# lorenlugosch/end-to-end-SLU

Measured on AMD Instinct MI355X. Metric: utterances/sec (train step, 3 s @16 kHz, B=64), higher is better.
Workload: dtype f32 (trainable stages: exact fp32 MFMA; convolutions and GRU contractions of FROZEN stages: bf16x3 = every fp32 operand split EXACTLY into 3 bf16 terms (3 x 8 = 24 significand bits, fp32's exponent range), 6 bf16 MFMA products per fp32 product (only terms below 2^-24 |a b| dropped), fp32 accumulatio; 1 GPU; experiments/no_unfreezing.cfg SLU train step (frozen SincNet/conv/biGRU encoder in train mode + intent biGRU trained): fwd + 3-slot CE + bwd + grad all-reduce + Adam; batch_per_gpu=64, global_batch=64, samples_per_utterance=48000, parallelism=dp1, encoder_lookahead_batches=20

## Files before the change

end-to-end-slu_amd/csrc/slu_head.hip:

```cpp
#include "slu_common.h"
#include "slu_philox.h"

#include <algorithm>

namespace slu {

constexpr int HEAD_THREADS = 256;
constexpr int HEAD_MAX_SLOTS = 8;

struct HeadParams {
  const float* h;
  const float* W;
  const float* bias;
  const long long* y;
  float* logits;
  int* argmax_t;
  long long* pred;
  float* d_logits;
  float* row_stats;
  float* loss_acc;
  double* epoch_sums;
  unsigned int* ticket;
  int T, B, C, V, S;
  int w_in_lds;
  int vec;
  float drop_p, drop_scale;
  unsigned long long seed, offset;
  const unsigned long long* offset_dev;
  float* h_drop;
  int slot_begin[HEAD_MAX_SLOTS + 1];
};

template <bool COHERENT>
__device__ __forceinline__ void head_reduce_body(const float* row_stats, float* loss_acc, double* epoch_sums, int B) {
  __shared__ float r0[256], r1[256];
  float a = 0.0f, c = 0.0f;
  for (int b = threadIdx.x; b < B; b += 256) {
    if (COHERENT) {
      const unsigned long long g = __hip_atomic_load(reinterpret_cast<const unsigned long long*>(row_stats) + b,
                                                     __ATOMIC_RELAXED, __HIP_MEMORY_SCOPE_AGENT);
      a += __uint_as_float((unsigned)(g & 0xffffffffull));
      c += __uint_as_float((unsigned)(g >> 32));
    } else {
      a += row_stats[2 * b]; c += row_stats[2 * b + 1];
    }
  }
  r0[threadIdx.x] = a; r1[threadIdx.x] = c;
  __syncthreads();
  for (int o = 128; o > 0; o >>= 1) {
    if ((int)threadIdx.x < o) { r0[threadIdx.x] += r0[threadIdx.x + o]; r1[threadIdx.x] += r1[threadIdx.x + o]; }
    __syncthreads();
  }
  if (threadIdx.x == 0) {
    const float loss = r0[0] / (float)B, acc = r1[0] / (float)B;
    loss_acc[0] = loss; loss_acc[1] = acc;
    if (epoch_sums) { epoch_sums[0] += (double)loss * (double)B; epoch_sums[1] += (double)acc * (double)B; }
  }
}

__global__ void __launch_bounds__(256)
head_reduce_kernel(const float* __restrict__ row_stats, float* __restrict__ loss_acc, double* epoch_sums, int B) {
  head_reduce_body<false>(row_stats, loss_acc, epoch_sums, B);
}

__global__ void __launch_bounds__(HEAD_THREADS)
head_fwd_kernel(const HeadParams p) {
  extern __shared__ __attribute__((aligned(16))) char smem[];
  float* sh = reinterpret_cast<float*>(smem);
  float* sw = sh + (size_t)p.T * (p.C + 1);
  float* sl = sw + (p.w_in_lds ? (size_t)p.V * (p.C + 1) : 0);
  float* sm = sl + (size_t)p.T * p.V;
  const int b = blockIdx.x, tid = threadIdx.x;
  const int T = p.T, C = p.C, V = p.V, LD = p.C + 1;
  if (p.vec) {
    const int C4 = C >> 2;
    const int nh = T * C4, nw = p.w_in_lds ? V * C4 : 0;
    const float thr = 1.0f - p.drop_p;
    const unsigned long long off = p.offset + (p.offset_dev ? *p.offset_dev : 0ull);
    constexpr int U = 13;
    for (int base = 0; base < nh + nw; base += HEAD_THREADS * U) {
      float4 v[U];
#pragma unroll
      for (int j = 0; j < U; ++j) {
        const int idx = base + j * HEAD_THREADS + tid;
        const bool ok = idx < nh + nw, isw = idx >= nh;
        const int e = ok ? (isw ? idx - nh : idx) : 0;
        const int row = e / C4, c = (e - row * C4) * 4;
        const float* src = (ok && isw) ? p.W + (size_t)row * C + c : p.h + ((size_t)row * p.B + b) * C + c;
        v[j] = *reinterpret_cast<const float4*>(src);
      }
#pragma unroll
      for (int j = 0; j < U; ++j) {
        const int idx = base + j * HEAD_THREADS + tid;
        const bool ok = idx < nh + nw, isw = idx >= nh;
        const int e = ok ? (isw ? idx - nh : idx) : 0;
        const int row = e / C4, c = (e - row * C4) * 4;
        if (!ok) continue;
        float4 x = v[j];
        if (!isw && p.drop_p > 0.0f) {
          const size_t g = ((size_t)row * p.B + b) * C + c;
          const float4 k = philox_keep4(p.seed, off, g, thr, p.drop_scale);
          x = make_float4(x.x * k.x, x.y * k.y, x.z * k.z, x.w * k.w);
          if (p.h_drop) *reinterpret_cast<float4*>(p.h_drop + g) = x;
        }
        float* dst = sh + (isw ? T + row : row) * LD + c;
        dst[0] = x.x; dst[1] = x.y; dst[2] = x.z; dst[3] = x.w;
      }
    }
  } else {
    const int nh = T * C, nw = p.w_in_lds ? V * C : 0;
    constexpr int U = 48;
    for (int base = 0; base < nh + nw; base += HEAD_THREADS * U) {
      float v[U];
#pragma unroll
      for (int j = 0; j < U; ++j) {
        const int idx = base + j * HEAD_THREADS + tid;
        const bool ok = idx < nh + nw, isw = idx >= nh;
        const int e = ok ? (isw ? idx - nh : idx) : 0;
        const int row = e / C, c = e - row * C;
        const float* src = (ok && isw) ? p.W + e : p.h + ((size_t)row * p.B + b) * C + c;
        v[j] = *src;
      }
#pragma unroll
      for (int j = 0; j < U; ++j) {
        const int idx = base + j * HEAD_THREADS + tid;
        const bool ok = idx < nh + nw, isw = idx >= nh;
        const int e = ok ? (isw ? idx - nh : idx) : 0;
        const int row = e / C, c = e - row * C;
        if (ok) sh[(isw ? T + row : row) * LD + c] = v[j];
      }
    }
  }
  __syncthreads();
  {
    const int lane = tid & 63, wave = tid >> 6;
    const int i = lane & 15, kg = lane >> 4;
    const int MT = (T + 15) >> 4, NT = (V + 15) >> 4;
    for (int tile = wave; tile < MT * NT; tile += HEAD_THREADS / 64) {
      const int mt = tile / NT, nt = tile - mt * NT;
      const float* a = sh + min(mt * 16 + i, T - 1) * LD + kg;
      const int vb = min(nt * 16 + i, V - 1);
      const float* w = (p.w_in_lds ? sw + vb * LD : p.W + (size_t)vb * C) + kg;
      f32x4 acc = {0.f, 0.f, 0.f, 0.f};
      int k0 = 0;
      for (; k0 + 31 < C; k0 += 32) {
        float av[8], bv[8];
#pragma unroll
        for (int u = 0; u < 8; ++u) { av[u] = a[k0 + 4 * u]; bv[u] = w[k0 + 4 * u]; }
#pragma unroll
        for (int u = 0; u < 8; ++u) acc = mfma16(av[u], bv[u], acc);
      }
      for (; k0 < C; k0 += 4) {
        const bool ok = k0 + kg < C;
        acc = mfma16(ok ? a[k0] : 0.0f, ok ? w[k0] : 0.0f, acc);
      }
#pragma unroll
      for (int r = 0; r < 4; ++r) {
        const int t = mt * 16 + 4 * kg + r, v = nt * 16 + i;
        if (t < T && v < V) sl[t * V + v] = acc[r] + p.bias[v];
      }
    }
  }
  __syncthreads();
  if (tid < V) {
    float best = sl[tid];
    int arg = 0;
    for (int t = 1; t < T; ++t) {
      const float x = sl[t * V + tid];
      if (x > best) { best = x; arg = t; }
    }
    sm[tid] = best;
    p.logits[(size_t)b * V + tid] = best;
    p.argmax_t[(size_t)b * V + tid] = arg;
  }
  __syncthreads();
  __shared__ float s_part[HEAD_THREADS];
  __shared__ int s_ok[HEAD_THREADS];
  if (tid < V) {
    int sl_ = 0;
    while (sl_ + 1 < p.S && tid >= p.slot_begin[sl_ + 1]) ++sl_;
    const int v0 = p.slot_begin[sl_], v1 = p.slot_begin[sl_ + 1];
    float mx = sm[v0];
    int am = v0;
    for (int v = v0 + 1; v < v1; ++v) if (sm[v] > mx) { mx = sm[v]; am = v; }
    if (tid == v0) p.pred[(size_t)b * p.S + sl_] = am - v0;
    s_part[tid] = 0.0f;
    s_ok[tid] = 1;
    if (p.y) {
      float den = 0.0f;
      for (int v = v0; v < v1; ++v) den += expf(sm[v] - mx);
      const int yv = (int)p.y[(size_t)b * p.S + sl_];
      if (tid == v0) {
        s_part[tid] = logf(den) - (sm[v0 + yv] - mx);
        s_ok[tid] = (am - v0 == yv) ? 1 : 0;
      }
      if (p.d_logits) {
        const float inv = 1.0f / (den * (float)p.B);
        p.d_logits[(size_t)b * V + tid] = expf(sm[tid] - mx) * inv - ((tid - v0 == yv) ? 1.0f / (float)p.B : 0.0f);
      }
    }
  }
  __syncthreads();
  if (tid == 0 && p.y) {
    float loss = 0.0f;
    bool all_ok = true;
    for (int s2 = 0; s2 < p.S; ++s2) {
      loss += s_part[p.slot_begin[s2]];
      all_ok = all_ok && (s_ok[p.slot_begin[s2]] != 0);
    }
    const unsigned long long g = (unsigned long long)__float_as_uint(loss) |
                                 ((unsigned long long)__float_as_uint(all_ok ? 1.0f : 0.0f) << 32);
    __hip_atomic_store(reinterpret_cast<unsigned long long*>(p.row_stats) + b, g, __ATOMIC_RELAXED, __HIP_MEMORY_SCOPE_AGENT);
  }
  if (p.ticket && p.y) {
    __shared__ int s_last;
    if (tid == 0) {
      asm volatile("s_waitcnt vmcnt(0)" ::: "memory");
      s_last = (__hip_atomic_fetch_add(p.ticket, 1u, __ATOMIC_RELAXED, __HIP_MEMORY_SCOPE_AGENT) == gridDim.x - 1) ? 1 : 0;
    }
    __syncthreads();
    if (s_last) {
      head_reduce_body<true>(p.row_stats, p.loss_acc, p.epoch_sums, p.B);
      if (tid == 0) *p.ticket = 0u;
    }
  }
}

struct HeadDrop {
  float p, scale;
  unsigned long long seed, offset;
  const unsigned long long* offset_dev;
};

__device__ __forceinline__ void
head_bwd_dh_body(char* smem, const int b, const float* __restrict__ d_logits, const int* __restrict__ argmax_t,
                 const float* __restrict__ W, const float* __restrict__ gscale,
                 float* __restrict__ d_h, int T, int B, int C, int V, const HeadDrop& dr) {
  float* acc = reinterpret_cast<float*>(smem);
  __shared__ float s_dl[HEAD_THREADS];
  __shared__ int s_at[HEAD_THREADS];
  const int tid = threadIdx.x;
  const float g = gscale[0];
  if (tid < V) { s_dl[tid] = d_logits[(size_t)b * V + tid] * g; s_at[tid] = argmax_t[(size_t)b * V + tid]; }
  for (int idx = tid; idx < T * C; idx += HEAD_THREADS) acc[idx] = 0.0f;
  __syncthreads();
  for (int c = tid; c < C; c += HEAD_THREADS)
    for (int v = 0; v < V; ++v) acc[s_at[v] * C + c] = fmaf(s_dl[v], W[(size_t)v * C + c], acc[s_at[v] * C + c]);
  __syncthreads();
  if (dr.p > 0.0f) {
    const int C4 = C >> 2;
    const float thr = 1.0f - dr.p;
    const unsigned long long off = dr.offset + (dr.offset_dev ? *dr.offset_dev : 0ull);
    for (int idx = tid; idx < T * C4; idx += HEAD_THREADS) {
      const int t = idx / C4, c = (idx - t * C4) * 4;
      const size_t g = ((size_t)t * B + b) * C + c;
      const float4 k = philox_keep4(dr.seed, off, g, thr, dr.scale);
      const float* a = acc + t * C + c;
      *reinterpret_cast<float4*>(d_h + g) = make_float4(a[0] * k.x, a[1] * k.y, a[2] * k.z, a[3] * k.w);
    }
    return;
  }
  for (int idx = tid; idx < T * C; idx += HEAD_THREADS) {
    const int t = idx / C, c = idx - t * C;
    d_h[((size_t)t * B + b) * C + c] = acc[idx];
  }
}

__device__ __forceinline__ void
head_bwd_dw_body(char* smem, const int v, const float* __restrict__ d_logits, const int* __restrict__ argmax_t,
                 const float* __restrict__ h, const float* __restrict__ gscale,
                 float* __restrict__ d_W, float* __restrict__ d_bias, int T, int B, int C, int V) {
  float* part = reinterpret_cast<float*>(smem);
  float* s_dl = part + 4 * C;
  int* s_at = reinterpret_cast<int*>(s_dl + HEAD_THREADS);
  __shared__ float s_b[4];
  const int lane = threadIdx.x & 63, w = threadIdx.x >> 6;
  const float g = gscale[0];
  float bsum = 0.0f;
  constexpr int KMAX = 16;
  float acc[KMAX];
#pragma unroll
  for (int k = 0; k < KMAX; ++k) acc[k] = 0.0f;
  for (int bb = 0; bb < B; bb += HEAD_THREADS) {
    __syncthreads();
    if (bb + (int)threadIdx.x < B) {
      s_dl[threadIdx.x] = d_logits[(size_t)(bb + threadIdx.x) * V + v];
      s_at[threadIdx.x] = argmax_t[(size_t)(bb + threadIdx.x) * V + v];
    }
    __syncthreads();
    const int nb = min(HEAD_THREADS, B - bb);
    for (int bl0 = w; bl0 < nb; bl0 += 32) {
      float hv[8][KMAX > 4 ? 4 : KMAX];
      if (C <= 256) {
#pragma unroll
        for (int u = 0; u < 8; ++u) {
          const int bl = min(bl0 + 4 * u, nb - 1);
          const float* hr = h + ((size_t)s_at[bl] * B + (bb + bl)) * C;
#pragma unroll
          for (int k = 0; k < 4; ++k) hv[u][k] = hr[min(lane + 64 * k, C - 1)];
        }
#pragma unroll
        for (int u = 0; u < 8; ++u) {
          const int bl = bl0 + 4 * u;
          if (bl < nb) {
            const float dl = s_dl[bl];
            bsum += dl;
#pragma unroll
            for (int k = 0; k < 4; ++k)
              if (lane + 64 * k < C) acc[k] = fmaf(dl, hv[u][k], acc[k]);
          }
        }
      } else {
        for (int u = 0; u < 8; ++u) {
          const int bl = bl0 + 4 * u;
          if (bl >= nb) break;
          const float dl = s_dl[bl];
          const float* hr = h + ((size_t)s_at[bl] * B + (bb + bl)) * C;
          bsum += dl;
#pragma unroll
          for (int k = 0; k < KMAX; ++k) {
            const int c = lane + 64 * k;
            if (c < C) acc[k] = fmaf(dl, hr[c], acc[k]);
          }
        }
      }
    }
  }
#pragma unroll
  for (int k = 0; k < KMAX; ++k) {
    const int c = lane + 64 * k;
    if (c < C) part[w * C + c] = acc[k];
  }
  if (lane == 0) s_b[w] = bsum;
  __syncthreads();
  for (int c = threadIdx.x; c < C; c += HEAD_THREADS)
    d_W[(size_t)v * C + c] = (((part[c] + part[C + c]) + part[2 * C + c]) + part[3 * C + c]) * g;
  if (threadIdx.x == 0) d_bias[v] = (((s_b[0] + s_b[1]) + s_b[2]) + s_b[3]) * g;
  (void)T;
}

__global__ void __launch_bounds__(HEAD_THREADS)
head_bwd_kernel(const float* __restrict__ d_logits, const int* __restrict__ argmax_t, const float* __restrict__ h,
                const float* __restrict__ W, const float* __restrict__ gscale, float* __restrict__ d_h,
                float* __restrict__ d_W, float* __restrict__ d_bias, int n_dh, int T, int B, int C, int V,
                const HeadDrop dr) {
  extern __shared__ __attribute__((aligned(16))) char smem[];
  if ((int)blockIdx.x < n_dh)
    head_bwd_dh_body(smem, blockIdx.x, d_logits, argmax_t, W, gscale, d_h, T, B, C, V, dr);
  else
    head_bwd_dw_body(smem, (int)blockIdx.x - n_dh, d_logits, argmax_t, h, gscale, d_W, d_bias, T, B, C, V);
}

}

using namespace slu;

extern "C" int slu_cls_maxpool_ce_fwd(const float* h, const float* weight, const float* bias,
                                      const int64_t* y, const int64_t* values_per_slot,
                                      int64_t num_slots, float* logits, int32_t* argmax_t,
                                      int64_t* pred, float* d_logits, float* row_stats,
                                      float* loss_acc, double* epoch_sums, uint32_t* ticket, float drop_p,
                                      uint64_t drop_seed, uint64_t drop_offset, const uint64_t* drop_offset_dev,
                                      float* h_drop, int64_t T, int64_t B, int64_t C, void* stream) {
  SLU_REQUIRE(h && weight && bias && logits && argmax_t && pred && values_per_slot, "slu_cls_maxpool_ce_fwd: null pointer");
  SLU_REQUIRE(drop_p >= 0.0f && drop_p < 1.0f, "slu_cls_maxpool_ce_fwd: dropout probability must be in [0, 1)");
  SLU_REQUIRE(num_slots >= 1 && num_slots <= HEAD_MAX_SLOTS, "slu_cls_maxpool_ce_fwd: 1..%d slots supported", HEAD_MAX_SLOTS);
  SLU_REQUIRE(!y || (row_stats && loss_acc), "slu_cls_maxpool_ce_fwd: row_stats / loss_acc required with labels");
  SLU_REQUIRE(T > 0 && B > 0 && C > 0, "slu_cls_maxpool_ce_fwd: non-positive size");
  HeadParams p;
  p.h = h; p.W = weight; p.bias = bias; p.y = (const long long*)y; p.logits = logits; p.argmax_t = argmax_t;
  p.pred = (long long*)pred; p.d_logits = d_logits; p.row_stats = row_stats;
  p.loss_acc = loss_acc; p.epoch_sums = y ? epoch_sums : nullptr; p.ticket = (unsigned int*)ticket;
  p.T = (int)T; p.B = (int)B; p.C = (int)C; p.S = (int)num_slots;
  p.vec = ((C & 3) == 0 && (((uintptr_t)h | (uintptr_t)weight | (uintptr_t)h_drop) & 15) == 0) ? 1 : 0;
  if (drop_p > 0.0f && !p.vec)
    SLU_FAIL(SLU_ERR_UNSUPPORTED, "slu_cls_maxpool_ce_fwd: the fused dropout needs C %% 4 == 0 (got %lld) and 16-byte aligned "
             "h / weight / h_drop", (long long)C);
  p.drop_p = drop_p; p.drop_scale = drop_p > 0.0f ? 1.0f / (1.0f - drop_p) : 1.0f;
  p.seed = drop_seed; p.offset = drop_offset; p.offset_dev = (const unsigned long long*)drop_offset_dev;
  p.h_drop = drop_p > 0.0f ? h_drop : nullptr;
  int V = 0;
  for (int s = 0; s < num_slots; ++s) { p.slot_begin[s] = V; V += (int)values_per_slot[s]; }
  p.slot_begin[num_slots] = V;
  p.V = V;
  SLU_REQUIRE(V >= 1 && V <= HEAD_THREADS, "slu_cls_maxpool_ce_fwd: 1..%d classifier outputs supported", HEAD_THREADS);
  size_t lds = ((size_t)(T + V) * (C + 1) + (size_t)T * V + V) * sizeof(float);
  p.w_in_lds = 1;
  const size_t lds_cap = 160 * 1024 - 4096;
  if (lds > lds_cap) {
    p.w_in_lds = 0;
    lds = ((size_t)T * (C + 1) + (size_t)T * V + V) * sizeof(float);
  }
  if (lds > lds_cap) SLU_FAIL(SLU_ERR_UNSUPPORTED, "slu_cls_maxpool_ce_fwd: T=%lld x C=%lld does not fit the LDS", (long long)T, (long long)C);
  if (lds > 64 * 1024) {
    hipError_t e = hipFuncSetAttribute((const void*)head_fwd_kernel, hipFuncAttributeMaxDynamicSharedMemorySize, (int)lds);
    if (e != hipSuccess) SLU_FAIL(SLU_ERR_HIP, "slu_cls_maxpool_ce_fwd: %s", hipGetErrorString(e));
  }
  hipStream_t st = (hipStream_t)stream;
  hipLaunchKernelGGL(head_fwd_kernel, dim3((unsigned)B), dim3(HEAD_THREADS), lds, st, p);
  SLU_CHECK_LAUNCH("head_fwd_kernel");
  if (y && !ticket) {
    hipLaunchKernelGGL(head_reduce_kernel, dim3(1), dim3(256), 0, st, (const float*)row_stats, loss_acc, epoch_sums, (int)B);
    SLU_CHECK_LAUNCH("head_reduce_kernel");
  }
  return SLU_OK;
}

extern "C" int slu_cls_maxpool_ce_bwd(const float* d_logits, const int32_t* argmax_t, const float* h,
                                      const float* weight, const float* grad_scale, float* d_h,
                                      float* d_weight, float* d_bias, float drop_p, uint64_t drop_seed,
                                      uint64_t drop_offset, const uint64_t* drop_offset_dev, int64_t T, int64_t B,
                                      int64_t C, int64_t V, void* stream) {
  SLU_REQUIRE(d_logits && argmax_t && h && weight && grad_scale, "slu_cls_maxpool_ce_bwd: null pointer");
  SLU_REQUIRE(drop_p >= 0.0f && drop_p < 1.0f, "slu_cls_maxpool_ce_bwd: dropout probability must be in [0, 1)");
  if (drop_p > 0.0f && d_h && ((C & 3) || ((uintptr_t)d_h & 15)))
    SLU_FAIL(SLU_ERR_UNSUPPORTED, "slu_cls_maxpool_ce_bwd: the fused dropout needs C %% 4 == 0 and a 16-byte aligned d_h");
  HeadDrop dr;
  dr.p = drop_p; dr.scale = drop_p > 0.0f ? 1.0f / (1.0f - drop_p) : 1.0f;
  dr.seed = drop_seed; dr.offset = drop_offset; dr.offset_dev = (const unsigned long long*)drop_offset_dev;
  SLU_REQUIRE((d_weight == nullptr) == (d_bias == nullptr), "slu_cls_maxpool_ce_bwd: d_weight and d_bias go together");
  SLU_REQUIRE(C <= 1024, "slu_cls_maxpool_ce_bwd: C <= 1024");
  hipStream_t st = (hipStream_t)stream;
  size_t lds = 0;
  if (d_h) {
    SLU_REQUIRE(V <= HEAD_THREADS && T * C * 4 <= 160 * 1024 - 4096, "slu_cls_maxpool_ce_bwd: T*C too large for the LDS");
    lds = (size_t)T * C * sizeof(float);
  }
  if (d_weight) lds = std::max(lds, ((size_t)4 * C + 2 * HEAD_THREADS) * sizeof(float));
  if (!d_h && !d_weight) return SLU_OK;
  if (lds > 64 * 1024) {
    hipError_t e = hipFuncSetAttribute((const void*)head_bwd_kernel, hipFuncAttributeMaxDynamicSharedMemorySize, (int)lds);
    if (e != hipSuccess) SLU_FAIL(SLU_ERR_HIP, "slu_cls_maxpool_ce_bwd: %s", hipGetErrorString(e));
  }
  const int n_dh = d_h ? (int)B : 0;
  hipLaunchKernelGGL(head_bwd_kernel, dim3((unsigned)(n_dh + (d_weight ? V : 0))), dim3(HEAD_THREADS), lds, st,
                     d_logits, argmax_t, h, weight, grad_scale, d_h, d_weight, d_bias, n_dh, (int)T, (int)B, (int)C, (int)V, dr);
  SLU_CHECK_LAUNCH("head_bwd_kernel");
  return SLU_OK;
}
```

Before: 376,700 utterances/s.

## Add fast head forward path with interleaved LDS layout and fused max-pool

Adds a templated fast variant of the classifier head forward kernel for small T, V and C. It stores h and W in LDS with a permuted, padded row layout so each lane can issue float4 loads feeding the fp32 MFMA. The loads are software-pipelined, and the max-over-time reduction is fused into the MFMA epilogue with cross-lane shuffles instead of writing the full T x V logits to LDS. The path is gated on shape conditions and can be turned off with an environment variable. This adds a second code path and assumes that at most two M tiles and two N tiles cover the work.

```diff
diff --git a/end-to-end-slu_amd/csrc/slu_head.hip b/end-to-end-slu_amd/csrc/slu_head.hip
--- a/end-to-end-slu_amd/csrc/slu_head.hip
+++ b/end-to-end-slu_amd/csrc/slu_head.hip
@@ -2,6 +2,7 @@
 #include "slu_philox.h"
 
 #include <algorithm>
+#include <cstdlib>
 
 namespace slu {
 
@@ -63,15 +64,17 @@
   head_reduce_body<false>(row_stats, loss_acc, epoch_sums, B);
 }
 
+template <bool FAST>
 __global__ void __launch_bounds__(HEAD_THREADS)
 head_fwd_kernel(const HeadParams p) {
   extern __shared__ __attribute__((aligned(16))) char smem[];
+  const int LD = FAST ? p.C + 4 : p.C + 1;
   float* sh = reinterpret_cast<float*>(smem);
-  float* sw = sh + (size_t)p.T * (p.C + 1);
-  float* sl = sw + (p.w_in_lds ? (size_t)p.V * (p.C + 1) : 0);
-  float* sm = sl + (size_t)p.T * p.V;
+  float* sw = sh + (size_t)p.T * LD;
+  float* sl = sw + (p.w_in_lds ? (size_t)p.V * LD : 0);
+  float* sm = sl + (FAST ? 128 : (size_t)p.T * p.V);
   const int b = blockIdx.x, tid = threadIdx.x;
-  const int T = p.T, C = p.C, V = p.V, LD = p.C + 1;
+  const int T = p.T, C = p.C, V = p.V;
   if (p.vec) {
     const int C4 = C >> 2;
     const int nh = T * C4, nw = p.w_in_lds ? V * C4 : 0;
@@ -103,8 +106,13 @@
           x = make_float4(x.x * k.x, x.y * k.y, x.z * k.z, x.w * k.w);
           if (p.h_drop) *reinterpret_cast<float4*>(p.h_drop + g) = x;
         }
-        float* dst = sh + (isw ? T + row : row) * LD + c;
-        dst[0] = x.x; dst[1] = x.y; dst[2] = x.z; dst[3] = x.w;
+        if (FAST) {
+          float* dst = sh + (isw ? T + row : row) * LD + (c & ~15) + ((c >> 2) & 3);
+          dst[0] = x.x; dst[4] = x.y; dst[8] = x.z; dst[12] = x.w;
+        } else {
+          float* dst = sh + (isw ? T + row : row) * LD + c;
+          dst[0] = x.x; dst[1] = x.y; dst[2] = x.z; dst[3] = x.w;
+        }
       }
     }
   } else {
@@ -132,7 +140,45 @@
     }
   }
   __syncthreads();
-  {
+  if (FAST) {
+    const int lane = tid & 63, wave = tid >> 6;
+    const int i = lane & 15, kg = lane >> 4;
+    const int MT = (T + 15) >> 4, NT = (V + 15) >> 4;
+    if (wave < MT * NT) {
+      const int mt = wave / NT, nt = wave - mt * NT;
+      const int vb = min(nt * 16 + i, V - 1);
+      const float4* a = reinterpret_cast<const float4*>(sh + min(mt * 16 + i, T - 1) * LD + 4 * kg);
+      const float4* w = reinterpret_cast<const float4*>(sw + vb * LD + 4 * kg);
+      const int nj = C >> 4;
+      f32x4 acc = {0.f, 0.f, 0.f, 0.f};
+      float4 a0 = a[0], w0 = w[0], a1 = a[4], w1 = w[4];
+      for (int j = 0; j < nj; j += 2) {
+        const int jn = min(j + 2, nj - 2);
+        const float4 a2 = a[4 * jn], w2 = w[4 * jn], a3 = a[4 * jn + 4], w3 = w[4 * jn + 4];
+        acc = mfma16(a0.x, w0.x, acc); acc = mfma16(a0.y, w0.y, acc); acc = mfma16(a0.z, w0.z, acc); acc = mfma16(a0.w, w0.w, acc);
+        acc = mfma16(a1.x, w1.x, acc); acc = mfma16(a1.y, w1.y, acc); acc = mfma16(a1.z, w1.z, acc); acc = mfma16(a1.w, w1.w, acc);
+        a0 = a2; w0 = w2; a1 = a3; w1 = w3;
+      }
+      const float bias = p.bias[vb];
+      float best = acc[0] + bias;
+      int arg = mt * 16 + 4 * kg;
+#pragma unroll
+      for (int r = 1; r < 4; ++r) {
+        const float x = acc[r] + bias;
+        if (x > best) { best = x; arg = mt * 16 + 4 * kg + r; }
+      }
+#pragma unroll
+      for (int o = 16; o < 64; o <<= 1) {
+        const float ob = __shfl_xor(best, o);
+        const int oa = __shfl_xor(arg, o);
+        if (ob > best || (ob == best && oa < arg)) { best = ob; arg = oa; }
+      }
+      if (kg == 0 && nt * 16 + i < V) {
+        sl[mt * 32 + nt * 16 + i] = best;
+        reinterpret_cast<int*>(sl)[64 + mt * 32 + nt * 16 + i] = arg;
+      }
+    }
+  } else {
     const int lane = tid & 63, wave = tid >> 6;
     const int i = lane & 15, kg = lane >> 4;
     const int MT = (T + 15) >> 4, NT = (V + 15) >> 4;
@@ -165,9 +211,14 @@
   if (tid < V) {
     float best = sl[tid];
     int arg = 0;
-    for (int t = 1; t < T; ++t) {
-      const float x = sl[t * V + tid];
-      if (x > best) { best = x; arg = t; }
+    if (FAST) {
+      arg = reinterpret_cast<const int*>(sl)[64 + tid];
+      if (T > 16 && sl[32 + tid] > best) { best = sl[32 + tid]; arg = reinterpret_cast<const int*>(sl)[96 + tid]; }
+    } else {
+      for (int t = 1; t < T; ++t) {
+        const float x = sl[t * V + tid];
+        if (x > best) { best = x; arg = t; }
+      }
     }
     sm[tid] = best;
     p.logits[(size_t)b * V + tid] = best;
@@ -386,18 +437,26 @@
   SLU_REQUIRE(V >= 1 && V <= HEAD_THREADS, "slu_cls_maxpool_ce_fwd: 1..%d classifier outputs supported", HEAD_THREADS);
   size_t lds = ((size_t)(T + V) * (C + 1) + (size_t)T * V + V) * sizeof(float);
   p.w_in_lds = 1;
+  bool fast = p.vec && (C & 31) == 0 && C <= 512 && T <= 32 && V <= 32;
+  if (fast) {
+    const char* env = getenv("SLU_HEAD_FAST");
+    fast = !(env && atoi(env) == 0);
+  }
+  if (fast) lds = ((size_t)(T + V) * (C + 4) + 128 + V) * sizeof(float);
   const size_t lds_cap = 160 * 1024 - 4096;
   if (lds > lds_cap) {
     p.w_in_lds = 0;
     lds = ((size_t)T * (C + 1) + (size_t)T * V + V) * sizeof(float);
   }
   if (lds > lds_cap) SLU_FAIL(SLU_ERR_UNSUPPORTED, "slu_cls_maxpool_ce_fwd: T=%lld x C=%lld does not fit the LDS", (long long)T, (long long)C);
+  const void* kernel = fast ? (const void*)head_fwd_kernel<true> : (const void*)head_fwd_kernel<false>;
   if (lds > 64 * 1024) {
-    hipError_t e = hipFuncSetAttribute((const void*)head_fwd_kernel, hipFuncAttributeMaxDynamicSharedMemorySize, (int)lds);
+    hipError_t e = hipFuncSetAttribute(kernel, hipFuncAttributeMaxDynamicSharedMemorySize, (int)lds);
     if (e != hipSuccess) SLU_FAIL(SLU_ERR_HIP, "slu_cls_maxpool_ce_fwd: %s", hipGetErrorString(e));
   }
   hipStream_t st = (hipStream_t)stream;
-  hipLaunchKernelGGL(head_fwd_kernel, dim3((unsigned)B), dim3(HEAD_THREADS), lds, st, p);
+  if (fast) hipLaunchKernelGGL(head_fwd_kernel<true>, dim3((unsigned)B), dim3(HEAD_THREADS), lds, st, p);
+  else hipLaunchKernelGGL(head_fwd_kernel<false>, dim3((unsigned)B), dim3(HEAD_THREADS), lds, st, p);
   SLU_CHECK_LAUNCH("head_fwd_kernel");
   if (y && !ticket) {
     hipLaunchKernelGGL(head_reduce_kernel, dim3(1), dim3(256), 0, st, (const float*)row_stats, loss_acc, epoch_sums, (int)B);
```

After: 377,200 utterances/s, median of 2. No clear change (+0.1%).
